# leonsick/s2d

Hardware: AMD Instinct MI355X
Metric: clip-frames/sec fwd+loss, R50 M2F-Video T=8 720p Q=100 (higher is better)
Workload: dtype f32 (f16x3 MFMA for dense contractions); 1 GPU; KDVideoMaskFormer fwd+loss (student+teacher fwd, GT+KD VideoSetCriterion), c4: 2 clips/GPU x T=8 x 720x1280, Q=100, P=160000, N=10 sparse GT instances/clip, encoder dropout 0.3; clips_per_gpu=2, frames_per_clip=8, parallelism=dp1 (clips sharded, no collective), streams=2

## Files before the change

### s2d_amd/csrc/gemm_bf16.hip

```cpp
#include "common.h"
#include "gemm_params.h"
#include "dropout.h"
#include <stdlib.h>
#include <type_traits>

namespace {

typedef __bf16 bf16x2 __attribute__((ext_vector_type(2)));
typedef __bf16 bf16x8 __attribute__((ext_vector_type(8)));
typedef float f32x2 __attribute__((ext_vector_type(2)));
typedef unsigned int u32x2 __attribute__((ext_vector_type(2)));
typedef unsigned int u32x4_t __attribute__((vector_size(16)));

constexpr int BN = 128, BK = 32, ROWW = 36;

__device__ __forceinline__ void split4(const f32x4 v, u32x2 &hi, u32x2 &lo)
{
    const f32x2 a = {v[0], v[1]}, b = {v[2], v[3]};
    const bf16x2 ha = __builtin_convertvector(a, bf16x2), hb = __builtin_convertvector(b, bf16x2);
    const unsigned int ua = __builtin_bit_cast(unsigned int, ha), ub = __builtin_bit_cast(unsigned int, hb);
    const f32x2 fa = {__uint_as_float(ua << 16), __uint_as_float(ua & 0xFFFF0000u)};
    const f32x2 fb = {__uint_as_float(ub << 16), __uint_as_float(ub & 0xFFFF0000u)};
    const bf16x2 la = __builtin_convertvector(a - fa, bf16x2), lb = __builtin_convertvector(b - fb, bf16x2);
    hi[0] = ua; hi[1] = ub;
// ... 1558 lines not shown
        for (int c = 0; c < CPI; ++c) {
            const int it = s.it0 + c < EPC ? s.it0 + c : EPC - 1;
#pragma unroll
            for (int w = 0; w < EV; ++w) v[c][w] = *reinterpret_cast<const f32x4 *>(epb + it * (ER * 68) + 4 * w);
        }
    };
    auto ep_write = [&](const EpSet &s, f32x4 (&v)[CPI][EV]) {
        if (s.it0 < 0 || s.it0 >= EPC) return;
        const bool cok = s.col < p.N;
#pragma unroll
        for (int c = 0; c < CPI; ++c) {
            const int it = s.it0 + c;
            if (it >= EPC) break;
            const int row = s.row + it * ER;
#pragma unroll
            for (int w = 0; w < EV; ++w) {
                if (CONV) v[c][w] *= s.sc[w];
                v[c][w] += s.bi[w];
            }
            if constexpr (DROP) {
                float m[8];
                s2d_dropout8((uint32_t)row + p.drop_row0, (uint32_t)(s.col >> 3), p.drop_stream, p.drop_k0, p.drop_k1, p.drop_thresh, p.drop_scale, m);
                v[c][0][0] *= m[0]; v[c][0][1] *= m[1]; v[c][0][2] *= m[2]; v[c][0][3] *= m[3];
                v[c][EV - 1][0] *= m[4]; v[c][EV - 1][1] *= m[5]; v[c][EV - 1][2] *= m[6]; v[c][EV - 1][3] *= m[7];
            }
#pragma unroll
            for (int w = 0; w < EV; ++w) {
                if (RES) {
#pragma unroll
                    for (int j = 0; j < 4; ++j) v[c][w][j] = __builtin_fmaf(s.rs[c][w][j], s.rmask[w], v[c][w][j]);
                }
#pragma unroll
                for (int j = 0; j < 4; ++j) v[c][w][j] = __builtin_amdgcn_fmed3f(v[c][w][j], relu_lo, __builtin_inff());
            }
            if (cok && row < p.M) {
#pragma unroll
                for (int w = 0; w < EV; ++w)
                    __builtin_amdgcn_raw_buffer_store_b128(__builtin_bit_cast(u32x4_t, v[c][w]), rsC, (int)s.coff, it * ldc4 + 16 * w, 0);
            }
        }
    };

    f32x4 ra[D][4], rb[D][4];
    unsigned int zm[D];
    EpSet es[D];
    set_tile(0);
#pragma unroll
    for (int d = 0; d < D; ++d) {
        load_set(ra[d], rb[d], zm[d]);
        ep_issue(es[d], false);
        __builtin_amdgcn_sched_barrier(0);
    }
    store_set(ra[0], rb[0], zm[0], 0);
    __builtin_amdgcn_sched_barrier(0);
    load_set(ra[0], rb[0], zm[0]);
    ep_issue(es[0], false);
    __builtin_amdgcn_sched_barrier(0);
    xkt = D; xtile = 0;
    __syncthreads();
    auto body = [&](int q, auto U) {
        constexpr int s = (decltype(U)::value + 1) % D;
        f32x4 ev[CPI][EV];
        ep_read(es[s], ev);
        __builtin_amdgcn_sched_barrier(0);
        store_set(ra[s], rb[s], zm[s], (q + 1) & 1);
        __builtin_amdgcn_sched_barrier(0);
        ep_write(es[s], ev);
        __builtin_amdgcn_sched_barrier(0);
        load_set(ra[s], rb[s], zm[s]);
        ep_issue(es[s], q + D < Q);
        __builtin_amdgcn_sched_barrier(0);
        __syncthreads();
    };
    using U0 = std::integral_constant<int, 0>;
    using U1 = std::integral_constant<int, 1>;
    using U2 = std::integral_constant<int, 2>;
    static_assert(D == 3, "the unrolled bodies below are written for three register sets");
    int q0 = 0;
    for (; q0 + D <= Q; q0 += D) { body(q0, U0{}); body(q0 + 1, U1{}); body(q0 + 2, U2{}); }
    if (q0 < Q) body(q0, U0{});
    if (q0 + 1 < Q) body(q0 + 1, U1{});
    __syncthreads();
    xtile = my_tiles;
    for (int it0 = 0; it0 < EPC; it0 += CPI) {
        xkt = it0 / CPI + 1;
        ep_issue(es[0], true);
        xtile = my_tiles;
        f32x4 ev[CPI][EV];
        ep_read(es[0], ev);
        ep_write(es[0], ev);
    }
}

template <bool CONV>
int launch_f16_hi(const GemmParams &p, int batch, hipStream_t st)
{
    const size_t lds = sizeof(float) * 4 * 64 * 36;
    const int nwg = cdiv(p.M, 128) * cdiv(p.N, 64);
    static int pre = -1;
    if (pre < 0) { const char *e = getenv("S2D_GEMM_HI_PRE"); pre = e ? atoi(e) : 1; }
    if (pre && p.Bsplit && p.res && !p.gate && p.K <= 4 * BK && ((p.N | p.ldc | p.ldr | p.res_cols) & 3) == 0)
        hipLaunchKernelGGL((gemm_f16x3_hi_kernel<CONV, true, true>), dim3(nwg, batch), dim3(256), lds, st, p);
    else if (p.Bsplit) hipLaunchKernelGGL((gemm_f16x3_hi_kernel<CONV, true>), dim3(nwg, batch), dim3(256), lds, st, p);
    else hipLaunchKernelGGL((gemm_f16x3_hi_kernel<CONV, false>), dim3(nwg, batch), dim3(256), lds, st, p);
    S2D_CHECK_LAUNCH();
    return S2D_OK;
}

template <bool CONV, bool PIPE, bool BSPLIT, bool DROP = false>
int launch_f16_v(const GemmParams &p, int batch, hipStream_t st)
{
    const size_t lds = sizeof(unsigned int) * 2 * (128 + BN) * ROWW;
    static S2dDevOnce attr_set;
    if (!attr_set.done()) {
        if (hipFuncSetAttribute(reinterpret_cast<const void *>(gemm_f16x3_kernel<CONV, PIPE, BSPLIT, DROP>),
                                hipFuncAttributeMaxDynamicSharedMemorySize, (int)lds) != hipSuccess)
            return S2D_ERR_LAUNCH;
        attr_set.mark();
    }
    const int nwg = cdiv(p.M, 128) * cdiv(p.N, BN);
    hipLaunchKernelGGL((gemm_f16x3_kernel<CONV, PIPE, BSPLIT, DROP>), dim3(nwg, batch), dim3(256), lds, st, p);
    S2D_CHECK_LAUNCH();
    return S2D_OK;
}

constexpr int WS_CONST_N = 16384;
__global__ void ws_constants_kernel(float *z, float *o)
{
    const int i = blockIdx.x * 256 + threadIdx.x;
    z[i] = 0.f; o[i] = 1.f;
}

int s2d_ws_constants(const float **zeros, const float **ones, hipStream_t st)
{
    static float *buf[16] = {};
    int dev = 0;
    if (hipGetDevice(&dev) != hipSuccess || dev < 0 || dev >= 16) return S2D_ERR_LAUNCH;
    if (!buf[dev]) {
        float *b = nullptr;
        if (hipMalloc(&b, sizeof(float) * 2 * WS_CONST_N) != hipSuccess) return S2D_ERR_LAUNCH;
        hipLaunchKernelGGL(ws_constants_kernel, dim3(WS_CONST_N / 256), dim3(256), 0, st, b, b + WS_CONST_N);
        if (hipStreamSynchronize(st) != hipSuccess) return S2D_ERR_LAUNCH;
        buf[dev] = b;
    }
    *zeros = buf[dev]; *ones = buf[dev] + WS_CONST_N;
    return S2D_OK;
}

template <bool CONV, bool BSPLIT, bool DROP, bool RES, bool ASPLIT = false>
int launch_f16_ws_v(const GemmParams &p, hipStream_t st)
{
    const size_t lds = sizeof(unsigned int) * 2 * (128 + BN) * ROWW + sizeof(float) * 4 * 64 * 68;
    static S2dDevOnce attr_set;
    static int cus = 0;
    if (!attr_set.done()) {
        if (hipFuncSetAttribute(reinterpret_cast<const void *>(gemm_f16x3_ws_kernel<CONV, BSPLIT, DROP, RES, ASPLIT>),
                                hipFuncAttributeMaxDynamicSharedMemorySize, (int)lds) != hipSuccess)
            return S2D_ERR_LAUNCH;
        int dev = 0;
        hipDeviceProp_t prop;
        if (hipGetDevice(&dev) != hipSuccess || hipGetDeviceProperties(&prop, dev) != hipSuccess) return S2D_ERR_LAUNCH;
        cus = prop.multiProcessorCount;
        attr_set.mark();
    }
    const int nwg = cdiv(p.M, 128) * cdiv(p.N, BN);
    GemmParams q = p;
    if (s2d_ws_constants(&q.zeros, &q.ones, st) != S2D_OK) return S2D_ERR_LAUNCH;
    hipLaunchKernelGGL((gemm_f16x3_ws_kernel<CONV, BSPLIT, DROP, RES, ASPLIT>), dim3(nwg < cus ? nwg : cus), dim3(512), lds, st, q);
    S2D_CHECK_LAUNCH();
    return S2D_OK;
}

template <bool CONV, bool BSPLIT, bool DROP>
int launch_f16_ws(const GemmParams &p, hipStream_t st)
{
    return p.res ? launch_f16_ws_v<CONV, BSPLIT, DROP, true>(p, st) : launch_f16_ws_v<CONV, BSPLIT, DROP, false>(p, st);
}

template <bool CONV, bool PIPE>
int launch_f16(const GemmParams &p, int batch, hipStream_t st)
{
    return p.Bsplit ? launch_f16_v<CONV, PIPE, true>(p, batch, st) : launch_f16_v<CONV, PIPE, false>(p, batch, st);
}

int launch_conv7x7s2_stem(const GemmParams &p, hipStream_t st)
{
    static int ph = -1;
    if (ph < 0) { const char *e = getenv("S2D_CONV_STEM_PH"); ph = e ? atoi(e) : 8; }
    const size_t lds16 = sizeof(float) * 4 * 64 * 68, lds8 = sizeof(float) * 4 * 32 * 68;
    static S2dDevOnce attr_set;
    if (!attr_set.done()) {
        if (hipFuncSetAttribute(reinterpret_cast<const void *>(conv7x7s2_c4_halo_kernel<16>), hipFuncAttributeMaxDynamicSharedMemorySize, (int)lds16) != hipSuccess)
            return S2D_ERR_LAUNCH;
        attr_set.mark();
    }
    const int imgs = p.M / (p.Hout * p.Wout);
    if (ph == 16) hipLaunchKernelGGL(conv7x7s2_c4_halo_kernel<16>, dim3(imgs * cdiv(p.Hout, 16) * cdiv(p.Wout, ST_P)), dim3(256), lds16, st, p);
    else hipLaunchKernelGGL(conv7x7s2_c4_halo_kernel<8>, dim3(imgs * cdiv(p.Hout, 8) * cdiv(p.Wout, ST_P)), dim3(256), lds8, st, p);
    S2D_CHECK_LAUNCH();
    return S2D_OK;
}

int launch_conv3x3_halo(const GemmParams &pin, hipStream_t st)
{
    const GemmParams &p = pin;
    int pipe = 0;
    if (const char *e = getenv("S2D_CONV_HALO_PIPE")) pipe = atoi(e);
    const size_t lds = sizeof(float) * 4 * 64 * 68;
    static S2dDevOnce attr_set;
    if (!attr_set.done()) {
        for (const void *fn : {reinterpret_cast<const void *>(conv3x3_f16x3_halo_kernel<8, 2, true>), reinterpret_cast<const void *>(conv3x3_f16x3_halo_kernel<16, 1, true>),
                               reinterpret_cast<const void *>(conv3x3_f16x3_halo_kernel<8, 2, false>), reinterpret_cast<const void *>(conv3x3_f16x3_halo_kernel<16, 1, false>)})
            if (hipFuncSetAttribute(fn, hipFuncAttributeMaxDynamicSharedMemorySize, (int)lds) != hipSuccess) return S2D_ERR_LAUNCH;
        attr_set.mark();
    }
    const int imgs = p.M / (p.Hin * p.Win);
    if (p.N <= 64) {
        const int nwg = imgs * cdiv(p.Hin, 16) * cdiv(p.Win, HT_W);
        if (pipe) hipLaunchKernelGGL((conv3x3_f16x3_halo_kernel<16, 1, true>), dim3(nwg), dim3(256), lds, st, p);
        else hipLaunchKernelGGL((conv3x3_f16x3_halo_kernel<16, 1, false>), dim3(nwg), dim3(256), lds, st, p);
    } else {
        const int nwg = imgs * cdiv(p.Hin, HT_H) * cdiv(p.Win, HT_W) * cdiv(p.N, BN);
        if (pipe) hipLaunchKernelGGL((conv3x3_f16x3_halo_kernel<8, 2, true>), dim3(nwg), dim3(256), lds, st, p);
        else hipLaunchKernelGGL((conv3x3_f16x3_halo_kernel<8, 2, false>), dim3(nwg), dim3(256), lds, st, p);
    }
    S2D_CHECK_LAUNCH();
    return S2D_OK;
}

template <bool CONV, bool BSPLIT>
int launch_w128_v(const GemmParams &p, int batch, hipStream_t st)
{
    const size_t lds = sizeof(float) * 4 * 64 * 68;
    static S2dDevOnce attr_set;
    if (!attr_set.done()) {
        if (hipFuncSetAttribute(reinterpret_cast<const void *>(gemm_bf16x3_w128_kernel<CONV, BSPLIT>),
                                hipFuncAttributeMaxDynamicSharedMemorySize, (int)lds) != hipSuccess)
            return S2D_ERR_LAUNCH;
        attr_set.mark();
    }
    const int nwg = cdiv(p.M, 256) * cdiv(p.N, BN);
    hipLaunchKernelGGL((gemm_bf16x3_w128_kernel<CONV, BSPLIT>), dim3(nwg, batch), dim3(256), lds, st, p);
    S2D_CHECK_LAUNCH();
    return S2D_OK;
}

template <bool CONV>
int launch_w128(const GemmParams &p, int batch, hipStream_t st)
{
    return p.Bsplit ? launch_w128_v<CONV, true>(p, batch, st) : launch_w128_v<CONV, false>(p, batch, st);
}

template <int WM, bool CONV>
int launch_t(const GemmParams &p, int batch, hipStream_t st)
{
    constexpr int BM = 64 * WM;
    const size_t lds = sizeof(unsigned int) * 2 * (BM + BN) * ROWW;
    static S2dDevOnce attr_set;
    if (!attr_set.done()) {
        if (hipFuncSetAttribute(reinterpret_cast<const void *>(gemm_bf16x3_kernel<WM, CONV>),
                                hipFuncAttributeMaxDynamicSharedMemorySize, (int)lds) != hipSuccess)
            return S2D_ERR_LAUNCH;
        attr_set.mark();
    }
    const int nwg = cdiv(p.M, BM) * cdiv(p.N, BN);
    hipLaunchKernelGGL((gemm_bf16x3_kernel<WM, CONV>), dim3(nwg, batch), dim3(128 * WM), lds, st, p);
    S2D_CHECK_LAUNCH();
    return S2D_OK;
}

template <bool BF16>
__global__ __launch_bounds__(256) void split_weights_kernel(const float *__restrict__ W, int N, int K, long ldw, int kblocks,
                                                            unsigned int *__restrict__ out, int vec4)
{
    const long i = (long)blockIdx.x * 256 + threadIdx.x;
    if (i >= (long)N * kblocks * 8) return;
    const int c4 = (int)(i & 7);
    const long nb = i >> 3;
    const int kb = (int)(nb % kblocks);
    const long n = nb / kblocks;
    const int k = kb * 32 + c4 * 4;
    f32x4 v = {0.f, 0.f, 0.f, 0.f};
    if (vec4) { if (k < K) v = *reinterpret_cast<const f32x4 *>(W + n * ldw + k); }
    else {
        float t[4] = {0.f, 0.f, 0.f, 0.f};
#pragma unroll
        for (int j = 0; j < 4; ++j)
            if (k + j < K) t[j] = W[n * ldw + k + j];
#pragma unroll
        for (int j = 0; j < 4; ++j) {
            float r;
            asm volatile("v_mov_b32 %0, %1" : "=v"(r) : "v"(t[j]));
            v[j] = r;
        }
    }
    u32x2 hi, lo;
    if (BF16) split4(v, hi, lo);
    else split4_f16(v, hi, lo);
    unsigned int *o = out + nb * 32;
    *reinterpret_cast<u32x2 *>(o + c4 * 2) = hi;
    *reinterpret_cast<u32x2 *>(o + 16 + c4 * 2) = lo;
}

}

int s2d_split_weights_launch(const float *W, int N, int K, long ldw, unsigned int *out, hipStream_t st, int bf16)
{
    const int kblocks = (K + 31) / 32;
    const long n = (long)N * kblocks * 8;
    if (n == 0) return S2D_OK;
    const int vec4 = ((K | ldw) & 3) == 0 && (reinterpret_cast<uintptr_t>(W) & 15) == 0;
    if (bf16) hipLaunchKernelGGL(split_weights_kernel<true>, dim3(cdiv(n, 256)), dim3(256), 0, st, W, N, K, ldw, kblocks, out, vec4);
    else hipLaunchKernelGGL(split_weights_kernel<false>, dim3(cdiv(n, 256)), dim3(256), 0, st, W, N, K, ldw, kblocks, out, vec4);
    S2D_CHECK_LAUNCH();
    return S2D_OK;
}

int s2d_launch_gemm_bf16x3(const GemmParams &pin, bool conv, int batch, hipStream_t st, int f16)
{
    GemmParams p = pin;
    const long bA = conv ? (long)(p.M / ((long)p.Hout * p.Wout)) * p.Hin * p.Win * p.Cin * 4L : ((long)(p.M - 1) * p.lda + p.K) * 4L;
    const long bB = ((long)(p.N - 1) * p.ldb + p.K) * 4L;
    if (bA > 0xFFFFFF00L || bB > 0xFFFFFF00L) return S2D_ERR_ARG;
    p.bytesA = (unsigned int)bA; p.bytesB = (unsigned int)bB;
    if (p.Bsplit) {
        if ((batch > 1 && p.sB != 0) || (long)p.N * ((p.K + 31) / 32) * 128L > 0xFFFFFF00L) return S2D_ERR_ARG;
        p.kblocks = (p.K + 31) / 32;
    }
    if (!f16 && (p.Asplit || p.gate || p.drop_thresh)) return S2D_ERR_ARG;
    if (s2d_gemm_small_m_ok(p, conv, batch, f16)) return s2d_launch_gemm_small_m(p, st);
    static int ws = -1;
    if (ws < 0) { const char *e = getenv("S2D_GEMM_WS"); ws = e ? atoi(e) : 0; }

    const long bC = ((long)(p.M - 1) * p.ldc + p.N) * 4L, bR = p.res ? ((long)((p.res_rows ? p.res_rows : p.M) - 1) * p.ldr + p.N) * 4L : 0;
    const bool ws_ok = ws && f16 && batch == 1 && !p.gate && p.N <= WS_CONST_N && (conv || !p.scale) && p.K >= 7 * BK - (BK - 1) && ((p.N | p.ldc | p.ldr | p.res_cols) & 3) == 0 &&
                       (conv ? (p.Cin % 4 == 0 && (p.Bsplit || p.K % BK == 0)) : p.K % BK == 0) &&
                       bC <= 0xFFFFFF00L && bR <= 0xFFFFFF00L && (!p.res_rows || p.res_rows >= 64) &&
                       (!p.drop_thresh || (((p.N | p.ldc) & 7) == 0 && (!p.res || ((p.ldr | p.res_cols) & 7) == 0)));
    if (p.Asplit) {
        const bool ok = f16 && !conv && batch == 1 && p.Bsplit && !p.scale && p.N <= WS_CONST_N && p.K >= 7 * BK - (BK - 1) && p.K % BK == 0 &&
                        ((p.N | p.ldc | p.ldr | p.res_cols) & 3) == 0 && bC <= 0xFFFFFF00L && bR <= 0xFFFFFF00L &&
                        (long)p.M * p.kblocks * 128L <= 0xFFFFFF00L && (!p.res_rows || p.res_rows >= 64) &&
                        (!p.drop_thresh || (((p.N | p.ldc) & 7) == 0 && (!p.res || ((p.ldr | p.res_cols) & 7) == 0)));
        if (!ok) return S2D_ERR_ARG;
        if (p.drop_thresh) return p.res ? launch_f16_ws_v<false, true, true, true, true>(p, st) : launch_f16_ws_v<false, true, true, false, true>(p, st);
        return p.res ? launch_f16_ws_v<false, true, false, true, true>(p, st) : launch_f16_ws_v<false, true, false, false, true>(p, st);
    }
    if (ws_ok && !conv && (ws == 2 || (p.Bsplit && (long)cdiv(p.M, 128) * cdiv(p.N, BN) >= 512))) {
        if (p.drop_thresh) return p.Bsplit ? launch_f16_ws<false, true, true>(p, st) : launch_f16_ws<false, false, true>(p, st);
        return p.Bsplit ? launch_f16_ws<false, true, false>(p, st) : launch_f16_ws<false, false, false>(p, st);
    }
    if (ws_ok && conv && !p.drop_thresh && (ws == 2 || (long)cdiv(p.M, 128) * cdiv(p.N, BN) >= 512)) {
        return p.Bsplit ? launch_f16_ws<true, true, false>(p, st) : launch_f16_ws<true, false, false>(p, st);
    }
    if (p.gate && (!f16 || batch != 1 || p.drop_thresh || ((p.N | p.ldc | p.ldr | p.res_cols | p.ldg) & 3))) return S2D_ERR_ARG;
    if (p.drop_thresh) {
        if (!f16 || conv || ((p.N | p.ldc) & 7) || (p.res && (((p.ldr | p.res_cols) & 7)))) return S2D_ERR_ARG;
        return p.Bsplit ? launch_f16_v<false, true, true, true>(p, batch, st) : launch_f16_v<false, true, false, true>(p, batch, st);
    }
    if (f16) {
        static int halo = -1;
        if (halo < 0) { const char *e = getenv("S2D_CONV_HALO"); halo = e ? atoi(e) : 1; }
        static int stem = -1;
        if (stem < 0) { const char *e = getenv("S2D_CONV_STEM"); stem = e ? atoi(e) : 1; }
        if (stem && conv && p.KH == 7 && p.KW == 7 && p.stride == 2 && p.pad == 3 && p.Cin == 4 && p.N <= 64 && p.N > 32 && p.Bsplit && batch == 1 &&
            ((p.N | p.ldc | p.ldr) & 3) == 0 && !p.res_rows && p.res_cols == p.N && !p.gate && (long)p.Hin * p.Win * 16L * (p.M / ((long)p.Hout * p.Wout)) < 0x7fffffffL)
            return launch_conv7x7s2_stem(p, st);
        static int halo64 = -1;
        if (halo64 < 0) { const char *e = getenv("S2D_CONV_HALO64"); halo64 = e ? atoi(e) : 1; }
        const int ph = p.N <= 64 ? 16 : HT_H;
        if (halo && conv && p.KH == 3 && p.KW == 3 && p.stride == 1 && p.pad == 1 && p.Cin % 32 == 0 && p.Bsplit && batch == 1 && (p.N > 64 || (halo64 && p.N > 32)) &&
            ((p.N | p.ldc | p.ldr) & 3) == 0 && !p.res_rows && p.res_cols == p.N && !p.gate &&
            (halo == 2 || (long)p.Hin * p.Win * 100 >= (long)cdiv(p.Hin, ph) * ph * cdiv(p.Win, HT_W) * HT_W * 88))
            return launch_conv3x3_halo(p, st);
        static int hi = -1;
        if (hi < 0) { const char *e = getenv("S2D_GEMM_HI"); hi = e ? atoi(e) : 2; }
        bool use_hi;
        if (hi != 2) use_hi = hi == 1;
        else if (conv && p.KH > 1) use_hi = p.N <= 64;
        else if (p.N <= 64 || p.K <= 128 || !p.Bsplit) use_hi = true;
        else if (p.K >= 512) use_hi = false;
        else {
            const float w128 = (float)(cdiv(p.N, 128) * 128) / p.N, w64 = (float)(cdiv(p.N, 64) * 64) / p.N;
            use_hi = w128 > w64 + 0.1f;
        }
        if (use_hi) return conv ? launch_f16_hi<true>(p, batch, st) : launch_f16_hi<false>(p, batch, st);
        static int pipe = -1;
        if (pipe < 0) { const char *e = getenv("S2D_GEMM_PIPE"); pipe = e ? atoi(e) : 1; }
        if (pipe) return conv ? launch_f16<true, true>(p, batch, st) : launch_f16<false, true>(p, batch, st);
        return conv ? launch_f16<true, false>(p, batch, st) : launch_f16<false, false>(p, batch, st);
    }
    static int w128 = -1;
    if (w128 < 0) { const char *e = getenv("S2D_GEMM_W128"); w128 = e ? atoi(e) : 1; }
    if (w128 && !conv && (long)cdiv(p.M, 256) * cdiv(p.N, BN) * batch >= (w128 == 2 ? 1 : 512)) return launch_w128<false>(p, batch, st);
    static int force = -1;
    if (force < 0) { const char *e = getenv("S2D_GEMM_WM"); force = e ? atoi(e) : 0; }
    bool big = (long)cdiv(p.M, 256) * cdiv(p.N, BN) * batch >= 256;
    if (force == 2) big = false;
    if (force == 4) big = true;
    if (big) return conv ? launch_t<4, true>(p, batch, st) : launch_t<4, false>(p, batch, st);
    return conv ? launch_t<2, true>(p, batch, st) : launch_t<2, false>(p, batch, st);
}
```

### s2d_amd/csrc/gemm_params.h

```cpp
#pragma once
#include <hip/hip_runtime.h>

struct GemmParams {
    const float *A, *B;
    float *C;
    int M, N, K;
    long lda, ldb, ldc;
    long sA, sB, sC;
    const float *scale, *bias, *res;
    long ldr, sR;
    int res_rows, res_cols;
    int relu;
    const float *gate;
    long ldg;
    float gate_scale;
    int Hin, Win, Cin, Hout, Wout, KH, KW, stride, pad;
    unsigned int bytesA, bytesB;
    const unsigned int *Bsplit;
    int kblocks;
    const unsigned int *Asplit;
    unsigned int drop_thresh;
    float drop_scale;
    unsigned int drop_k0, drop_k1, drop_stream;
    unsigned int drop_row0;
    const float *zeros, *ones;
};


int s2d_split_weights_launch(const float *W, int N, int K, long ldw, unsigned int *out, hipStream_t st, int bf16);
int s2d_launch_gemm_bf16x3(const GemmParams &p, bool conv, int batch, hipStream_t st, int f16);
bool s2d_gemm_small_m_ok(const GemmParams &p, bool conv, int batch, int f16);
int s2d_launch_gemm_small_m(const GemmParams &p, hipStream_t st);
```

Measured before the change: 174.7 clip-frames/s.

## Add A-stationary f16x3 GEMM kernel for short-K large-M matmuls

Adds a GEMM kernel for K of 64, 128 or 256 in which each wave loads its 32 A rows once, splits them into hi/lo f16 pairs held in registers, and then sweeps over a range of N tiles, streaming only the pre-split B through double-buffered LDS. Columns are divided across blocks so that roughly two blocks per CU are launched. This removes the repeated A loading and splitting that the generic tiled kernel does for every N tile. By default it is used only for K=256 GEMMs with no residual and a large M*N. The cost is high register pressure from keeping the split A in registers, and the dispatch condition uses getenv on every call without caching the result.

```diff
diff --git a/s2d_amd/csrc/gemm_astat.hip b/s2d_amd/csrc/gemm_astat.hip
--- /dev/null
+++ b/s2d_amd/csrc/gemm_astat.hip
@@ -0,0 +1,193 @@
+#include "common.h"
+#include "gemm_params.h"
+#include <stdlib.h>
+
+namespace {
+
+typedef float f32x2 __attribute__((ext_vector_type(2)));
+typedef unsigned int u32x4 __attribute__((ext_vector_type(4)));
+typedef __fp16 h16x2 __attribute__((ext_vector_type(2)));
+typedef _Float16 f16x8 __attribute__((ext_vector_type(8)));
+
+constexpr int BM = 128, BNT = 64, ROWW = 36, EPW = 68;
+constexpr int PLANE = BNT * ROWW + 32;
+constexpr int STAGE = 2 * PLANE;
+constexpr size_t LDS_BYTES = sizeof(unsigned int) * 2 * STAGE + sizeof(float) * 4 * 32 * EPW;
+
+__device__ __forceinline__ void split8(const f32x4 a, const f32x4 b, f16x8 &hi, f16x8 &lo)
+{
+    u32x4 h, l;
+    const f32x4 v[2] = {a, b};
+#pragma unroll
+    for (int i = 0; i < 2; ++i) {
+        const h16x2 h0 = __builtin_amdgcn_cvt_pkrtz(v[i][0], v[i][1]), h1 = __builtin_amdgcn_cvt_pkrtz(v[i][2], v[i][3]);
+        const f32x2 x0 = {v[i][0], v[i][1]}, x1 = {v[i][2], v[i][3]};
+        const f32x2 r0 = (x0 - __builtin_convertvector(h0, f32x2)) * 2048.f, r1 = (x1 - __builtin_convertvector(h1, f32x2)) * 2048.f;
+        const h16x2 l0 = __builtin_amdgcn_cvt_pkrtz(r0[0], r0[1]), l1 = __builtin_amdgcn_cvt_pkrtz(r1[0], r1[1]);
+        h[2 * i] = __builtin_bit_cast(unsigned int, h0); h[2 * i + 1] = __builtin_bit_cast(unsigned int, h1);
+        l[2 * i] = __builtin_bit_cast(unsigned int, l0); l[2 * i + 1] = __builtin_bit_cast(unsigned int, l1);
+    }
+    hi = __builtin_bit_cast(f16x8, h);
+    lo = __builtin_bit_cast(f16x8, l);
+}
+
+template <int KB>
+__global__ __launch_bounds__(256, 2) void gemm_f16x3_astat_kernel(GemmParams p, int nsplit, int cpw)
+{
+    constexpr int NST = KB / 2;
+    extern __shared__ __attribute__((aligned(16))) unsigned int lds[];
+    unsigned int *Bs = lds;
+    const int tid = threadIdx.x, lane = tid & 63, wave = tid >> 6;
+    float *ep = reinterpret_cast<float *>(lds + 2 * STAGE) + wave * 32 * EPW;
+    const int l32 = lane & 31, h = lane >> 5;
+    const int c16 = lane & 15, rr = lane >> 4;
+    const int tiles_n = (p.N + BNT - 1) / BNT;
+    const int tile_m = blockIdx.x / nsplit, part = blockIdx.x % nsplit;
+    const int m0 = tile_m * BM + wave * 32;
+    const int ct0 = part * cpw, ct1 = min(ct0 + cpw, tiles_n);
+    constexpr unsigned int OOB = 0xFFFFFFF0u;
+    const __amdgpu_buffer_rsrc_t rsA = __builtin_amdgcn_make_buffer_rsrc(const_cast<float *>(p.A), 0, (int)p.bytesA, 0x00020000);
+    const __amdgpu_buffer_rsrc_t rsB =
+        __builtin_amdgcn_make_buffer_rsrc(const_cast<unsigned int *>(p.Bsplit), 0, (int)((long)p.N * KB * 128L), 0x00020000);
+
+    const int bcol = tid >> 4, bw = tid & 15;
+    const unsigned int b_lds = ((bw >> 3) * PLANE + bcol * ROWW + (bw & 7) * 4);
+    constexpr int DIST = NST % 2 == 0 ? 2 : 1;
+    u32x4 rb[DIST][4];
+    auto load_stage = [&](int set, int ct, int kc) {
+#pragma unroll
+        for (int i = 0; i < 4; ++i) {
+            const int n = ct * BNT + bcol + 16 * i;
+            const unsigned int off = n < p.N ? (unsigned int)(((long)n * KB + 2 * kc) * 128L + bw * 16) : OOB;
+            rb[set][i] = __builtin_bit_cast(u32x4, __builtin_amdgcn_raw_buffer_load_b128(rsB, (int)off, 0, 0));
+        }
+    };
+    auto store_stage = [&](int set, int buf) {
+#pragma unroll
+        for (int i = 0; i < 4; ++i) *reinterpret_cast<u32x4 *>(&Bs[buf * STAGE + b_lds + 16 * i * ROWW]) = rb[set][i];
+    };
+    load_stage(0, ct0, 0);
+    if constexpr (DIST == 2) load_stage(1, ct0, 1);
+
+    f16x8 ah[2 * KB], al[2 * KB];
+#pragma unroll
+    for (int c = 0; c < NST; ++c) {
+        f32x4 t[8];
+#pragma unroll
+        for (int it = 0; it < 8; ++it) {
+            const int row = m0 + it * 4 + rr;
+            const unsigned int off = row < p.M ? (unsigned int)(((long)row * p.lda + c * 64 + c16 * 4) * 4L) : OOB;
+            t[it] = __builtin_bit_cast(f32x4, __builtin_amdgcn_raw_buffer_load_b128(rsA, (int)off, 0, 0));
+        }
+#pragma unroll
+        for (int it = 0; it < 8; ++it) *reinterpret_cast<f32x4 *>(&ep[(it * 4 + rr) * EPW + c16 * 4]) = t[it];
+#pragma unroll
+        for (int s = 0; s < 4; ++s) {
+            const f32x4 a = *reinterpret_cast<const f32x4 *>(&ep[l32 * EPW + 16 * s + 8 * h]);
+            const f32x4 b = *reinterpret_cast<const f32x4 *>(&ep[l32 * EPW + 16 * s + 8 * h + 4]);
+            split8(a, b, ah[c * 4 + s], al[c * 4 + s]);
+        }
+    }
+    store_stage(0, 0);
+    __syncthreads();
+
+    f32x16 accm[2], accx[2];
+#pragma unroll
+    for (int j = 0; j < 2; ++j)
+#pragma unroll
+        for (int r = 0; r < 16; ++r) { accm[j][r] = 0.f; accx[j][r] = 0.f; }
+
+    int buf = 0;
+    for (int ct = ct0; ct < ct1; ++ct) {
+#pragma unroll
+        for (int kc = 0; kc < NST; ++kc) {
+            const bool more = kc + 1 < NST || ct + 1 < ct1;
+            {
+                const int ctn = ct + (kc + DIST >= NST ? 1 : 0);
+                if (ctn < ct1) load_stage(kc % DIST, ctn, (kc + DIST) % NST);
+            }
+            const unsigned int *bs = &Bs[buf * STAGE + l32 * ROWW + 4 * h];
+#pragma unroll
+            for (int q = 0; q < 4; ++q) {
+                const unsigned int *bq = bs + (q >> 1) * PLANE + 8 * (q & 1);
+                const f16x8 bh0 = *reinterpret_cast<const f16x8 *>(bq), bl0 = *reinterpret_cast<const f16x8 *>(bq + 16);
+                const f16x8 bh1 = *reinterpret_cast<const f16x8 *>(bq + 32 * ROWW), bl1 = *reinterpret_cast<const f16x8 *>(bq + 32 * ROWW + 16);
+                const f16x8 a_h = ah[kc * 4 + q], a_l = al[kc * 4 + q];
+                accx[0] = __builtin_amdgcn_mfma_f32_32x32x16_f16(a_l, bh0, accx[0], 0, 0, 0);
+                accx[1] = __builtin_amdgcn_mfma_f32_32x32x16_f16(a_l, bh1, accx[1], 0, 0, 0);
+                accm[0] = __builtin_amdgcn_mfma_f32_32x32x16_f16(a_h, bh0, accm[0], 0, 0, 0);
+                accx[0] = __builtin_amdgcn_mfma_f32_32x32x16_f16(a_h, bl0, accx[0], 0, 0, 0);
+                accx[1] = __builtin_amdgcn_mfma_f32_32x32x16_f16(a_h, bl1, accx[1], 0, 0, 0);
+                accm[1] = __builtin_amdgcn_mfma_f32_32x32x16_f16(a_h, bh1, accm[1], 0, 0, 0);
+            }
+            if (more) store_stage((kc + 1) % DIST, buf ^ 1);
+            __syncthreads();
+            buf ^= 1;
+        }
+#pragma unroll
+        for (int tn = 0; tn < 2; ++tn)
+#pragma unroll
+            for (int r = 0; r < 16; ++r) {
+                ep[((r & 3) + 8 * (r >> 2) + 4 * h) * EPW + tn * 32 + l32] = accm[tn][r] + accx[tn][r] * (1.0f / 2048.0f);
+                accm[tn][r] = 0.f; accx[tn][r] = 0.f;
+            }
+        const int col = ct * BNT + c16 * 4;
+        if (col < p.N) {
+            f32x4 sc = {1.f, 1.f, 1.f, 1.f}, bi = {0.f, 0.f, 0.f, 0.f};
+            if (p.scale) sc = *reinterpret_cast<const f32x4 *>(p.scale + col);
+            if (p.bias) bi = *reinterpret_cast<const f32x4 *>(p.bias + col);
+#pragma unroll 4
+            for (int it = 0; it < 8; ++it) {
+                const int row = m0 + rr + it * 4;
+                if (row >= p.M) break;
+                f32x4 v = *reinterpret_cast<const f32x4 *>(&ep[(it * 4 + rr) * EPW + c16 * 4]);
+                v = v * sc + bi;
+                if (p.res && col < p.res_cols) v += *reinterpret_cast<const f32x4 *>(p.res + (long)(p.res_rows ? row % p.res_rows : row) * p.ldr + col);
+                if (p.relu) { v[0] = fmaxf(v[0], 0.f); v[1] = fmaxf(v[1], 0.f); v[2] = fmaxf(v[2], 0.f); v[3] = fmaxf(v[3], 0.f); }
+                *reinterpret_cast<f32x4 *>(p.C + (long)row * p.ldc + col) = v;
+            }
+        }
+    }
+}
+
+template <int KB>
+int launch_astat(const GemmParams &p, hipStream_t st)
+{
+    static S2dDevOnce attr_set;
+    static int cus = 0;
+    if (!attr_set.done()) {
+        if (hipFuncSetAttribute(reinterpret_cast<const void *>(gemm_f16x3_astat_kernel<KB>), hipFuncAttributeMaxDynamicSharedMemorySize,
+                                (int)LDS_BYTES) != hipSuccess)
+            return S2D_ERR_LAUNCH;
+        int dev = 0;
+        hipDeviceProp_t prop;
+        if (hipGetDevice(&dev) != hipSuccess || hipGetDeviceProperties(&prop, dev) != hipSuccess) return S2D_ERR_LAUNCH;
+        cus = prop.multiProcessorCount;
+        attr_set.mark();
+    }
+    const int tiles_m = cdiv(p.M, BM), tiles_n = cdiv(p.N, BNT);
+    int nsplit = cdiv(2 * cus, tiles_m);
+    nsplit = nsplit < 1 ? 1 : nsplit > tiles_n ? tiles_n : nsplit;
+    const int cpw = cdiv(tiles_n, nsplit);
+    nsplit = cdiv(tiles_n, cpw);
+    hipLaunchKernelGGL(gemm_f16x3_astat_kernel<KB>, dim3(tiles_m * nsplit), dim3(256), LDS_BYTES, st, p, nsplit, cpw);
+    S2D_CHECK_LAUNCH();
+    return S2D_OK;
+}
+
+}
+
+bool s2d_gemm_astat_ok(const GemmParams &p, bool conv, int batch, int f16)
+{
+    return f16 && !conv && batch == 1 && p.Bsplit && !p.Asplit && !p.gate && !p.drop_thresh && (p.K == 64 || p.K == 128 || p.K == 256) &&
+           p.N > BNT && ((p.lda | p.N | p.ldc | p.ldr | p.res_cols) & 3) == 0 &&
+           ((reinterpret_cast<uintptr_t>(p.A) | reinterpret_cast<uintptr_t>(p.C) | reinterpret_cast<uintptr_t>(p.res) |
+             reinterpret_cast<uintptr_t>(p.scale) | reinterpret_cast<uintptr_t>(p.bias)) & 15) == 0;
+}
+
+int s2d_launch_gemm_astat(const GemmParams &p, hipStream_t st)
+{
+    if (p.K == 64) return launch_astat<2>(p, st);
+    if (p.K == 128) return launch_astat<4>(p, st);
+    return launch_astat<8>(p, st);
+}
diff --git a/s2d_amd/csrc/gemm_bf16.hip b/s2d_amd/csrc/gemm_bf16.hip
--- a/s2d_amd/csrc/gemm_bf16.hip
+++ b/s2d_amd/csrc/gemm_bf16.hip
@@ -1884,6 +1884,11 @@
     *reinterpret_cast<u32x2 *>(o + 16 + c4 * 2) = lo;
 }
 
+bool s2d_gemm_astat_wins(const GemmParams &p)
+{
+    return p.K == 256 && !p.res && (long)p.M * p.N >= 58880L * 1024;
+}
+
 }
 
 int s2d_split_weights_launch(const float *W, int N, int K, long ldw, unsigned int *out, hipStream_t st, int bf16)
@@ -1955,6 +1960,9 @@
             ((p.N | p.ldc | p.ldr) & 3) == 0 && !p.res_rows && p.res_cols == p.N && !p.gate &&
             (halo == 2 || (long)p.Hin * p.Win * 100 >= (long)cdiv(p.Hin, ph) * ph * cdiv(p.Win, HT_W) * HT_W * 88))
             return launch_conv3x3_halo(p, st);
+        int astat = 1;
+        if (const char *e = getenv("S2D_GEMM_ASTAT")) astat = atoi(e);
+        if (astat && s2d_gemm_astat_ok(p, conv, batch, f16) && (astat == 2 || s2d_gemm_astat_wins(p))) return s2d_launch_gemm_astat(p, st);
         static int hi = -1;
         if (hi < 0) { const char *e = getenv("S2D_GEMM_HI"); hi = e ? atoi(e) : 2; }
         bool use_hi;
diff --git a/s2d_amd/csrc/gemm_params.h b/s2d_amd/csrc/gemm_params.h
--- a/s2d_amd/csrc/gemm_params.h
+++ b/s2d_amd/csrc/gemm_params.h
@@ -31,3 +31,5 @@
 int s2d_launch_gemm_bf16x3(const GemmParams &p, bool conv, int batch, hipStream_t st, int f16);
 bool s2d_gemm_small_m_ok(const GemmParams &p, bool conv, int batch, int f16);
 int s2d_launch_gemm_small_m(const GemmParams &p, hipStream_t st);
+bool s2d_gemm_astat_ok(const GemmParams &p, bool conv, int batch, int f16);
+int s2d_launch_gemm_astat(const GemmParams &p, hipStream_t st);
```

After: 175.4 clip-frames/s, median of 6. About the same (+0.4%).
